# Aditya-Somasi/Vision-Inspection-System

Hardware: AMD Instinct MI355X
Metric: inspected images/sec (1024x1024, Qwen2-VL-7B) (higher is better)
Workload: dtype bf16; 1 GPU; configs[1]: Qwen2-VL-7B Inspector bf16, single 1024x1024 image per step per GPU, greedy decode 128 tok; batch=1, image_px=1024, weights=seeded random bf16 at exact 7B shapes, parallelism=dp1 (whole images)

## Files before the change

### include/vis_hip.h

```cpp
#ifndef VIS_HIP_H
#define VIS_HIP_H

#ifdef __cplusplus
extern "C" {
#endif

typedef void* vis_stream_t;

#define VIS_OK 0
#define VIS_ERR_ARG 1
#define VIS_ERR_LAUNCH 2
#define VIS_ERR_UNSUPPORTED 3

#define VIS_ACT_NONE 0
#define VIS_ACT_QUICKGELU 1
#define VIS_ACT_GELU_ERF 2
#define VIS_ACT_SWIGLU 3

int vis_abi_version(void);

int vis_gemm_bf16(const void* A, const void* W, const void* bias, const void* R, void* C,
                  int M, int N, int K, int lda, int ldw, int ldc, int ldr, int act, vis_stream_t stream);

int vis_rmsnorm_bf16(const void* x, const void* w, void* y, int rows, int N, int ldx, int ldy,
// ... 53 lines not shown

int vis_decode_attn_parts(const void* part, int ksplit, int slab_rows, const void* bias, const void* sx, const void* sw,
                          const void* cos_t, const void* sin_t, void* k_cache, void* v_cache, const void* step_ptr,
                          void* part_o, void* part_ml, void* out, int Hq, int Hkv, int HD, int cache_tokens, int nsplit,
                          float scale, int batch, long long cache_bs, long long tab_bs, int shared_len, vis_stream_t stream);

int vis_decode_attn_forked(const void* qkv, const void* cos_t, const void* sin_t, void* k_cache, void* v_cache,
                           const void* step_ptr, void* part_o, void* part_ml, void* out, int Hq, int Hkv, int HD,
                           int cache_tokens, int nsplit, float scale, int batch, long long qkv_bs, long long cache_bs,
                           long long tab_bs, const int* parent, const int* fork_len, vis_stream_t stream);
int vis_decode_attn_parts_forked(const void* part, int ksplit, int slab_rows, const void* bias, const void* sx, const void* sw,
                                 const void* cos_t, const void* sin_t, void* k_cache, void* v_cache, const void* step_ptr,
                                 void* part_o, void* part_ml, void* out, int Hq, int Hkv, int HD, int cache_tokens, int nsplit,
                                 float scale, int batch, long long cache_bs, long long tab_bs, const int* parent,
                                 const int* fork_len, vis_stream_t stream);

int vis_decode_chain_sync_ints(void);
long long vis_decode_chain_ws_bytes(int Hq, int Hkv, int nsplit);
int vis_decode_chain_ctx_limit(int Hq, int Hkv, int K);
int vis_decode_chain(const void* x, const void* x_idx, int x_rows, const void* Wqkv, const void* bqkv, const void* norm_w, const void* Wo, void* y,
                     const void* cos_t, const void* sin_t, void* k_cache, void* v_cache, const void* step_ptr,
                     void* ws, void* sync, int Hq, int Hkv, int HD, int K, int ldw_qkv, int ldw_o,
                     int cache_tokens, int nsplit, int ctx_bound, float scale, float eps, vis_stream_t stream);

int vis_gemv_bf16_argmax(const void* x, const void* W, const void* norm_w, void* logits, int N, int K, int ldw, float eps,
                         void* ws_val, void* ws_idx, void* tokens, int max_tokens, void* cur_token, void* step_ptr,
                         float inv_temp, unsigned seed, vis_stream_t stream);

int vis_argmax_f32(const void* logits, int V, void* ws_val, void* ws_idx, void* tokens, int max_tokens,
                   void* cur_token, void* step_ptr, float inv_temp, unsigned seed, int batch, int ld_logits,
                   vis_stream_t stream);

long long vis_logprobs_ws_bytes(int V, int batch);
int vis_logprobs_f32(const void* logits, int V, int ld_logits, const void* tokens, int max_tokens, const void* step_ptr,
                     int top_k, void* lp, void* top_ids, void* ws, long long ws_bytes, int batch, vis_stream_t stream);

int vis_json_mask(void* state, const void* tokens, int max_tokens, const void* step_ptr, const void* tok_off,
                  const void* tok_bytes, const void* tok_flags, const void* eos_ids, int n_eos, int V, void* allow,
                  int ld_allow, int batch, vis_stream_t stream);
int vis_schema_mask(void* state, const void* tokens, int max_tokens, const void* step_ptr, const void* tok_off,
                    const void* tok_bytes, const void* tok_flags, const void* eos_ids, int n_eos, int V, void* allow,
                    int ld_allow, const void* header, const void* trans, const void* byte_class, const void* state_flags,
                    int cap_states, int cap_classes, int batch, vis_stream_t stream);
int vis_argmax_masked_f32(const void* logits, int V, void* ws_val, void* ws_idx, void* tokens, int max_tokens,
                          void* cur_token, void* step_ptr, float inv_temp, unsigned seed, int batch, int ld_logits,
                          const void* allow, int ld_allow, vis_stream_t stream);
// ... 212 lines not shown
```

### vision-inspection-system_amd/decode_stage.py

```python
from __future__ import annotations

import logging
import os
import threading
from typing import Dict, List, NamedTuple, Optional, Sequence

import torch

from . import hip, spec
from .fork import check_fork_tables, fork_layout
from .pick import PickStage

_LOG = logging.getLogger("vision_inspection_system_amd.engine")

_CHAIN_LOCKS_GUARD = threading.Lock()
_CHAIN_ORDER_LOCKS: Dict[Optional[int], threading.Lock] = {}
_CHAIN_LAST: Dict[Optional[int], "torch.cuda.Event"] = {}


def _chain_order_lock(index: Optional[int]) -> threading.Lock:
    with _CHAIN_LOCKS_GUARD:
        return _CHAIN_ORDER_LOCKS.setdefault(index, threading.Lock())


class DecodeLayer(NamedTuple):
    w: object
    q8: Optional[dict]
    q4: Optional[dict]
    cross: bool
    idx: int
    bias: Optional[torch.Tensor]


_GEMV = {"bf16": "gemv", "fp8": "gemv_fp8", "mxfp4": "gemv_mxfp4"}


def _wt(L: DecodeLayer, name: str, fmt: str) -> tuple:
    return (getattr(L.w, name),) if fmt == "bf16" else (L.q8 if fmt == "fp8" else L.q4)[name]


class DecodeStage(PickStage):

    def _init_decode_stage(self, layers: Sequence[DecodeLayer], norm_w: torch.Tensor, lm_head: torch.Tensor,
                           q8_head: Optional[tuple] = None, q4_head: Optional[tuple] = None) -> None:
        self.dec_layers: List[DecodeLayer] = list(layers)
        self.dec_norm_w = norm_w
        self.dec_head = {"bf16": (lm_head,), "fp8": q8_head, "mxfp4": q4_head}
        self.dec_n_self = sum(1 for L in self.dec_layers if not L.cross)
        self._init_pick_stage()
        self.fork_on = False
        self.fork_parent_b: Optional[torch.Tensor] = None
        self.fork_len_b: Optional[torch.Tensor] = None
        self._spec: Optional[spec.SpecBuffers] = None
        self._spec_cfg: Optional[spec.SpecConfig] = None
        self._spec_pred = False
        self._spec_graphs: Dict[tuple, torch.cuda.CUDAGraph] = {}

    def _attn_share(self, B: int, shared: int) -> dict:
        if self.fork_on:
            return dict(fork=(self.fork_parent_b[:B], self.fork_len_b[:B]))
        return dict(shared_len=shared)

    def _fork_model_state(self, root: int, child: int) -> None:
        """Hook: copy what the model keeps per slot besides the self KV cache (rope rows, cross-attention keys) from ``root``
        into ``child``."""

    def _fork_choices(self, roots: Sequence[Optional[int]], n: Sequence[int], prefix_len: int, seeds, penalties,
                      shaping) -> List[Optional[List[int]]]:
        live = [j for j in range(len(roots)) if roots[j] is not None]
        lay = fork_layout([self.slot_prompt_len[roots[j]] for j in live], [n[j] for j in live], prefix_len, self.max_batch)
        out: List[Optional[List[int]]] = [None] * len(roots)
        for i, j in enumerate(live):
            if roots[j] != i:
                raise RuntimeError("prompt passes did not fill consecutive slots")
            out[j] = lay.slots[i]
        for child, root, lo, hi in lay.copies:
            j = live[root]
            self.kcache_b[child][:, :, lo:hi].copy_(self.kcache_b[root][:, :, lo:hi])
            self.vcache_b[child][:, :, lo:hi].copy_(self.vcache_b[root][:, :, lo:hi])
# ... 86 lines not shown
                    continue
                q = qkv[..., :Hq * D]
                proj(x, _wt(L, "qkv_w", fmt), q, norm_w=lw.ln1_w, eps=eps)
                self._decode_cross_attn(L, q, att, B)
                proj(att, _wt(L, "o_w", fmt), x2, residual=x)
            else:
                kc, vc = (self.kcache_b[:B, L.idx], self.vcache_b[:B, L.idx]) if B else (self.kcache[L.idx], self.vcache[L.idx])
                if chained:
                    try:
                        hip.decode_chain(self.w.embed if li == 0 else x, lw.qkv_w, L.bias, lw.ln1_w, lw.o_w, x2, cos, sin, kc, vc,
                                         step, self.chain_ws, self.chain_sync, Hq, Hkv, D, self.nsplit, scale, eps,
                                         x_index=cur if li == 0 else None, ctx_bound=self.chain_ctx_limit)
                    except hip.ChainRefused as e:
                        if li:
                            raise
                        _LOG.warning("%s - decoding on the four launches per layer head (VIS_MAX_CTX=%d)", e, self.max_ctx)
                        self.chain_sync, self._chain_state, chained = None, None, False
                        hip.gather_rows(self.w.embed, cur, self.d_x)
                if not chained:
                    proj(x, _wt(L, "qkv_w", fmt), qkv, bias=L.bias, norm_w=lw.ln1_w, eps=eps)
                    hip.decode_attn(qkv, cos, sin, kc, vc, step, self.part_o, self.part_ml, att, Hq, Hkv, D, self.nsplit, scale,
                                    **(self._attn_share(B, shared) if B else {}))
                    proj(att, _wt(L, "o_w", fmt), x2, residual=x)
            proj(x2, _wt(L, "gateup_w", fmt), act, norm_w=lw.ln2_w, act=hip.ACT_SWIGLU, eps=eps)
            proj(act, _wt(L, "down_w", fmt), x, residual=x2)
        if chained:
            self._gemv_pick(x, *self.dec_head["bf16"], logits, self.ws_val, self.ws_idx, tokens, cur, step,
                            norm_w=self.dec_norm_w, eps=eps, temperature=self.temperature, seed=self.seed)
        else:
            proj(x, self.dec_head[fmt], logits, norm_w=self.dec_norm_w, eps=eps)
            self._pick(logits, self.ws_val, self.ws_idx, tokens, cur, step, self.temperature, self.seed)
        self._logprobs_after_pick(B or 1)
        self._stop_after_pick(B or 1)
        self._stream_after_pick(B or 1)

    def _spec_begin(self, cfg: "spec.SpecConfig", max_new_tokens: int,
                    prediction: Optional[Sequence[int]] = None) -> "spec.SpecBuffers":
        cross = self.dec_n_self != len(self.dec_layers)
        if cross and not self.speculative_supported:
            raise ValueError("speculative decoding is not supported on a model with cross-attention layers unless its engine "
                             "was built for it (MllamaEngine(.., speculative=True))")
        spec.check_rows_fit(self.cfg, cfg.rows)
        if cross:
            spec.check_cross_rows_fit(self.cfg, cfg.rows)
        if self._spec is None:
            self._spec = spec.SpecBuffers(self.cfg, max(self.nsplit, self.xsplit) if cross else self.nsplit, self.max_ctx,
# ... 265 lines not shown
        g = torch.cuda.CUDAGraph()
        with torch.cuda.graph(g, capture_error_mode="thread_local"):
            step_fn()
        if len(cache) >= capacity:
            cache.pop(next(iter(cache)))
        cache[key] = g
        return g

    def _decode_steps(self, n_steps: int, use_graph: bool, chained: bool = False) -> None:
        if use_graph:
            g = self._ensure_graph(chained=chained)
            if chained and self.chain_sync is None:
                g = self._ensure_graph(chained=False)
            for _ in range(n_steps):
                g.replay()
        else:
            for _ in range(n_steps):
                self._decode_step(chained)

    def _decode_ordered(self, n_steps: int, use_graph: bool) -> None:
        base = self.prompt_len + self._decoded
        self._decoded += n_steps
        n_chain = max(0, min(n_steps, self.chain_ctx_limit - base)) if self.chain_sync is not None else 0
        if n_chain:
            self._chain_epoch_guard(n_chain)
            with _chain_order_lock(self.device.index):
                cur = torch.cuda.current_stream(self.device)
                prev = _CHAIN_LAST.get(self.device.index)
                if prev is not None:
                    cur.wait_event(prev)
                self._decode_steps(n_chain, use_graph, True)
                ev = torch.cuda.Event()
                ev.record(cur)
                _CHAIN_LAST[self.device.index] = ev
        if n_steps > n_chain:
            self._decode_steps(n_steps - n_chain, use_graph, False)

    def _chain_epoch_guard(self, n_steps: int) -> None:
        self._chain_launches += n_steps * self.dec_n_self
        if self._chain_launches >= (1 << 31):
            self.chain_sync.zero_()
            self.chain_ws.zero_()
            self._chain_launches = n_steps * self.dec_n_self

    def generated(self, n: int) -> List[int]:
        s = self.prompt_len - 1
        toks = self.tokens[s:s + n].cpu().tolist()
        self.check_chain()
        return toks

    def check_chain(self) -> None:
        if self.chain_sync is not None and int(self.chain_sync[hip.CHAIN_STATUS_WORD].item()) != 0:
            self.chain_sync.zero_()
            self.chain_ws.zero_()
            self._chain_launches = 0
            raise hip.ChainStalled("vis_decode_chain: a hand-off wait inside the launch timed out (decode results invalid)")
```

### vision-inspection-system_amd/engine.py

```python
from __future__ import annotations

import collections
import logging
import os
import threading
from typing import Dict, List, Optional, Sequence, Tuple

import numpy as np
import torch

from . import hip
from .decode_stage import DecodeLayer
from .generation import Generation
from .request import Switches
from .config import Qwen2VLConfig
from .weights import DeviceWeights, PATCH_K_PAD


def _round_up(x: int, m: int) -> int:
    return (x + m - 1) // m * m


def vision_pos_hw(grids: Sequence[Tuple[int, int, int]], merge: int) -> np.ndarray:
    out = []
# ... 788 lines not shown
    def shared_prefix_len(self, id_lists: Sequence[Sequence[int]]) -> int:
        if len(id_lists) < 2 or os.environ.get("VIS_SHARE_PREFIX", "1") == "0":
            return 0
        cfg = self.cfg
        first = np.asarray(list(id_lists[0]), dtype=np.int64)
        P = len(first) - 1
        for ids in id_lists[1:]:
            other = np.asarray(list(ids), dtype=np.int64)
            m = min(P, len(other) - 1)
            neq = np.nonzero(first[:m] != other[:m])[0]
            P = int(neq[0]) if neq.size else m
        special = np.nonzero((first[:P] == cfg.image_token_id) | (first[:P] == cfg.vision_start_id))[0]
        if special.size:
            P = int(special[0])
        P = (P // 64) * 64
        return P if P >= self.min_shared_prefix else 0

    def _decode_rope(self, B: int) -> tuple:
        return self.cos_b[:B], self.sin_b[:B], self.batch_shared_len

    def _ensure_graph(self, batch: int = 0, chained: bool = False) -> torch.cuda.CUDAGraph:
        fork = bool(batch) and self.fork_on
        key = (self.temperature, self.seed, batch, self.batch_shared_len if batch and not fork else 0,
               bool(chained) and not batch, fork) + self._pick_key() + self._stop_key() + self._shape_key() + self._stream_key() + self._ban_key()
        return self._captured_step(self._graphs, 8, key, batch, chained)

    def decode(self, n_steps: int, use_graph: bool = True) -> None:
        if self.prompt_len + n_steps + 1 > self.max_ctx:
            raise ValueError("decode would overflow the KV cache")
        if self.prompt_len + self._decoded + n_steps > self.decode_limit:
            raise ValueError("decode beyond the rope rows prepared by prefill (pass max_new_tokens)")
        self._decode_ordered(n_steps, use_graph)

    def disable_chain(self) -> None:
        if self.chain_sync is not None:
            self._chain_state = (self.chain_ws, self.chain_sync)
        self.chain_sync = None
        self._chain_clean_requests = 0
        self._graphs.clear()

    def _maybe_reenable_chain(self) -> None:
        if self.chain_sync is not None or self._chain_state is None:
            return
        self._chain_clean_requests += 1
        retry_after = int(os.environ.get("VIS_CHAIN_RETRY_AFTER", "64"))
        if retry_after > 0 and self._chain_clean_requests >= retry_after:
            self.chain_ws, self.chain_sync = self._chain_state
# ... 42 lines not shown
```

### vision-inspection-system_amd/generation.py

```python
from __future__ import annotations

import logging
from dataclasses import replace
from typing import List, Sequence

import torch

from . import hip, spec
from .ban import check_ban
from .decode_stage import DecodeStage
from .fork import check_n_list
from .json_mode import JsonModeError, check_schema
from .logprobs import check_k
from .penalties import check_penalties
from .request import Switches
from .sampling import check_seeds, check_top_p
from .shaping import check_shaping
from .stop import check_stop

_LOG = logging.getLogger("vision_inspection_system_amd.engine")


class Generation(DecodeStage):

# ... 23 lines not shown
        pred = spec.check_prediction_ids(sw.prediction, getattr(self, "max_ctx", None))
        sp = spec.with_prediction(sw.speculative, pred is not None)
        if sp is not None:
            what = "speculative" if pred is None else "prediction (speculative decoding)"
            if not self.speculative_supported:
                raise ValueError(("speculative decoding is" if pred is None else "prediction (speculative decoding) is") +
                                 " offered by the Qwen2-VL / Qwen2.5-VL engine only, unless an MllamaEngine is built for it: "
                                 "MllamaEngine(.., speculative=True), or VIS_AUDITOR_SPECULATIVE=k (1..3) where the client "
                                 "loads it")
            spec.check_exclusive(sp, temperature, seed, what=what, **sw.exclusive())
        penalties = check_penalties(sw.repetition_penalty, sw.frequency_penalty, sw.presence_penalty, 1)
        shaping = check_shaping(sw.top_k, sw.min_p, sw.logit_bias, 1)
        ban = check_ban(sw.no_repeat_ngram_size, sw.bad_words, sw.min_tokens, 1, max_new_tokens, json_mode=sw.json_mode,
                        json_schema=sw.json_schema)
        with self._pick_request(sw.logprobs, sw.json_mode, sw.json_schema, sw.top_p, False, penalties, stop=sw.stop,
                                shaping=shaping, on_stream=sw.on_stream, **({} if ban is None else {"ban": ban})):
            self.stop_eos = not ignore_eos
            self._stream_bind([[0]])
            max_new_tokens = self._clamp_request(input_ids, max_new_tokens)
            if sp is not None:
                return self._run_single_spec(sp, input_ids, frames, max_new_tokens, ignore_eos, use_graph, check_every, pred, temperature, seed)
            try:
                out = self._run_single(input_ids, frames, max_new_tokens, ignore_eos, use_graph, check_every, temperature, seed)
                self._maybe_reenable_chain()
                return out
            except hip.ChainStalled as e:
                _LOG.warning("%s - continuing on the unchained decode step", e)
                self.disable_chain()
                return self._run_single(input_ids, frames, max_new_tokens, ignore_eos, use_graph, check_every, temperature, seed)

    def _run_single(self, input_ids, frames, max_new_tokens, ignore_eos, use_graph, check_every, temperature, seed) -> List[int]:
        ev = [torch.cuda.Event(enable_timing=True) for _ in range(3)]
        ev[0].record()
        self._prompt_pass(input_ids, frames, max_new_tokens, temperature, seed)
        ev[1].record()
        max_new_tokens = min(max_new_tokens, self.max_ctx - len(input_ids) - 1)
        done, eos = 1, set(self.cfg.eos_ids)
        while done < max_new_tokens and not self._stream_cancelled():
            if self.stop_on:
                if self._stop_done([0]):
                    break
            elif not ignore_eos and any(t in eos for t in self.generated(done)):
                break
            n = min(check_every if not ignore_eos or self.stop_on else max_new_tokens, max_new_tokens - done)
            self.decode(n, use_graph=use_graph)
            done += n
        ev[2].record()
# ... 157 lines not shown
```

### vision-inspection-system_amd/hip.py

```python
from __future__ import annotations

import ctypes
import os
from typing import Optional, Sequence

import torch

_CSRC = os.path.join(os.path.dirname(os.path.abspath(__file__)), "csrc")
LIB_PATH = os.environ.get("VIS_HIP_LIB") or os.path.join(_CSRC, "libvis_hip.so")

ACT_NONE, ACT_QUICKGELU, ACT_GELU_ERF, ACT_SWIGLU = 0, 1, 2, 3
DECODE_KEYS_PER_SPLIT = 64

_SIGS = {
    "vis_abi_version": "",
    "vis_gemm_bf16": "ppppp" + "iiiiiiii" + "p",
    "vis_gemm_bf16_splitk": "pppppp" + "iiiiiiiii" + "p",
    "vis_gemm_bf16_splitk_part": "ppp" + "iiiiii" + "p",
    "vis_splitk_finalize_norm": "p" + "i" + "pppppp" + "iiiii" + "f" + "p",
    "vis_gemm_fp8": "pppppppp" + "iiiiiiiii" + "p",
    "vis_gemm_bf16_plan": "iiiiiiii" + "p" + "i",
    "vis_gemm_fp8_plan": "iiiiiiiii" + "p" + "i",
    "vis_quant_rows_fp8": "ppppp" + "iiii" + "f" + "p",
    "vis_rmsnorm_bf16": "ppp" + "iiii" + "f" + "p",
# ... 5 lines not shown
    "vis_attn_prefill_rows": "ppppp" + "iiiiiiiii" + "f" + "i" + "p",
    "vis_attn_prefill_rows_many": "ppppp" + "iiiiiiiii" + "f" + "i" + "i" + "lll" + "p" + "p",
    "vis_attn_prefill_pairs": "ppppp" + "iiiiiiii" + "f" + "i" + "p",
    "vis_attn_prefill_pairs_many": "ppppp" + "iiiiiiii" + "f" + "i" + "i" + "lll" + "p" + "p",
    "vis_attn_split_ws_bytes": "ii",
    "vis_attn_prefill_split": "ppppp" + "iiiiiiii" + "f" + "i" + "p" + "l" + "p",
    "vis_gemv_bf16": "pppppp" + "iiiii" + "f" + "p",
    "vis_gemv_fp8w": "ppppppp" + "iiiii" + "f" + "p",
    "vis_gemv_bf16_rows": "pppppp" + "iiiiiiiii" + "f" + "p",
    "vis_gemv_fp8w_rows": "ppppppp" + "iiiiiiiii" + "f" + "p",
    "vis_gemv_mxfp4w": "ppppppp" + "iiiiii" + "f" + "p",
    "vis_gemv_mxfp4w_rows": "ppppppp" + "iiiiiiiiii" + "f" + "p",
    "vis_gemm_decode_mxfp4_ksplit": "ii",
    "vis_gemm_decode_mxfp4": "ppppp" + "iiiiiiiii" + "p",
    "vis_decode_attn": "ppppppppp" + "iiiii" + "f" + "i" + "lll" + "p",
    "vis_decode_attn_shared": "ppppppppp" + "iiiii" + "f" + "i" + "lll" + "i" + "p",
    "vis_decode_attn_parts": "p" + "ii" + "p" * 11 + "iiiii" + "f" + "i" + "ll" + "i" + "p",
    "vis_decode_attn_forked": "ppppppppp" + "iiiii" + "f" + "i" + "lll" + "pp" + "p",
    "vis_decode_attn_parts_forked": "p" + "ii" + "p" * 11 + "iiiii" + "f" + "i" + "ll" + "pp" + "p",
    "vis_decode_chain_sync_ints": "",
    "vis_decode_chain_ws_bytes": "iii",
    "vis_decode_chain_ctx_limit": "iii",
    "vis_decode_chain": "ppi" + "p" * 12 + "i" * 9 + "ff" + "p",
    "vis_gemv_bf16_argmax": "pppp" + "iii" + "f" + "ppp" + "i" + "pp" + "fu" + "p",
    "vis_argmax_f32": "p" + "i" + "ppp" + "i" + "pp" + "fu" + "ii" + "p",
    "vis_logprobs_ws_bytes": "ii",
    "vis_logprobs_f32": "p" + "ii" + "p" + "i" + "p" + "i" + "ppp" + "l" + "i" + "p",
    "vis_json_mask": "pp" + "i" + "p" * 5 + "iip" + "ii" + "p",
    "vis_schema_mask": "pp" + "i" + "p" * 5 + "iip" + "i" + "pppp" + "iii" + "p",
    "vis_argmax_masked_f32": "p" + "i" + "ppp" + "i" + "pp" + "fu" + "ii" + "p" + "i" + "p",
    "vis_gemv_bf16_argmax_masked": "pppp" + "iii" + "f" + "ppp" + "i" + "pp" + "fu" + "p" + "p",
    "vis_sample_ws_bytes": "ii",
    "vis_sample_f32": "p" + "ii" + "p" + "i" + "ff" + "pp" + "i" + "pp" + "i" + "pp" + "p",
    "vis_penalty_state_bytes": "ii",
    "vis_penalty_prompt": "pi" + "pi" + "p",
    "vis_penalize_f32": "p" + "ii" + "ppp" + "i" + "pp" + "ii" + "p",
    "vis_shape_ws_bytes": "ii",
    "vis_shape_f32": "p" + "ii" + "p" + "i" + "ppppp" + "p" + "i" + "pp" + "i" + "p",
    "vis_ban_f32": "p" + "ii" + "p" + "i" + "pp" + "i" + "pppppp" + "i" + "p" + "i" + "p" + "ii" + "p",
    "vis_decode_attn_draft": "ppppppppp" + "iiiii" + "f" + "i" + "l" + "p",
    "vis_decode_cross_attn_draft": "pppppppp" + "iiiii" + "ff" + "il" + "p",
    "vis_decode_cross_attn_fp8_draft": "pppppppppp" + "iiiii" + "ff" + "il" + "p",
    "vis_spec_accept": "p" + "iii" + "pppppp" + "i" + "ppp" + "p",
    "vis_spec_accept_sampled": "p" + "iii" + "pppppp" + "i" + "ppp" + "p" + "p",
    "vis_spec_accept_masked": "p" + "iii" + "pppppp" + "i" + "ppp" + "p" + "pi" + "p",
    "vis_schema_mask_rows": "pp" + "i" + "ppp" + "i" + "pppp" + "ii" + "p" + "i" + "pppp" + "ii" + "p",
# ... 113 lines not shown
    global _CALL_TRACE
    tr, _CALL_TRACE = _CALL_TRACE, None
    return tr or {}


def exported_symbols() -> list:
    return list(_SIGS)


def load() -> ctypes.CDLL:
    global _lib
    if _lib is not None:
        return _lib
    if not os.path.exists(LIB_PATH):
        raise HipLibraryError(
            f"{LIB_PATH} not found: build it with `make -C {_CSRC}` (or __graft_entry__.build()); "
            "this package has no CPU fallback")
    lib = ctypes.CDLL(LIB_PATH)
    for name, sig in _SIGS.items():
        fn = getattr(lib, name)
        fn.restype = ctypes.c_int
        fn.argtypes = [_CT[c] for c in sig]
    lib.vis_decode_chain_ws_bytes.restype = ctypes.c_longlong
    lib.vis_decode_proj_ws_bytes.restype = ctypes.c_longlong
    lib.vis_logprobs_ws_bytes.restype = ctypes.c_longlong
    lib.vis_sample_ws_bytes.restype = ctypes.c_longlong
    lib.vis_penalty_state_bytes.restype = ctypes.c_longlong
    lib.vis_shape_ws_bytes.restype = ctypes.c_longlong
    _lib = _Lib(lib)
    return _lib


def _check(rc: int, name: str) -> None:
    if rc != 0:
        why = {1: "argument/shape/alignment precondition violated", 2: "HIP launch error",
               3: "shape not covered by this kernel form on this device"}.get(rc, "unknown")
        raise HipLibraryError(f"{name} failed with status {rc} ({why})")


def _ptr(t: Optional[torch.Tensor]) -> Optional[int]:
    if t is None:
        return None
    if not t.is_cuda:
        raise HipLibraryError("device tensor required (no CPU path exists)")
    return t.data_ptr()

# ... 810 lines not shown
    if qkv_w.shape != (nq, K) or qkv_w.stride(1) != 1 or o_w.shape != (K, n_q * head_dim) or o_w.stride(1) != 1 \
            or norm_w.numel() != K or y.numel() != K or (qkv_b is not None and qkv_b.numel() != nq):
        raise HipLibraryError("decode_chain: bad projection shapes")
    if k_cache.dim() != 3 or k_cache.shape[0] != n_kv or k_cache.shape[2] != head_dim or v_cache.shape != k_cache.shape \
            or not k_cache.is_contiguous() or not v_cache.is_contiguous():
        raise HipLibraryError("decode_chain: bad cache shape")
    T = k_cache.shape[1]
    if cos_t.shape != (T, head_dim) or sin_t.shape != cos_t.shape or cos_t.dtype != torch.float32 or not cos_t.is_contiguous() \
            or not sin_t.is_contiguous() or step.dtype != torch.int32 or step.numel() != 1:
        raise HipLibraryError("decode_chain: bad tables / step")
    lib = load()
    if ws.dtype != torch.int64 or ws.numel() * 8 < lib.vis_decode_chain_ws_bytes(n_q, n_kv, nsplit) \
            or sync.dtype != torch.int32 or sync.numel() < lib.vis_decode_chain_sync_ints():
        raise HipLibraryError("decode_chain: workspace too small")
    rc = lib.vis_decode_chain(_ptr(x), _ptr(x_index), x_rows, _ptr(qkv_w), _ptr(qkv_b), _ptr(norm_w), _ptr(o_w), _ptr(y), _ptr(cos_t), _ptr(sin_t),
                              _ptr(k_cache), _ptr(v_cache), _ptr(step), _ptr(ws), _ptr(sync), n_q, n_kv, head_dim, K,
                              qkv_w.stride(0), o_w.stride(0), T, nsplit, ctx_bound, scale, eps, _stream())
    if rc == 3:
        raise ChainRefused(f"vis_decode_chain: {n_q}/{n_kv} heads, hidden {K}, {nsplit} context splits are outside the chained "
                           "form on this device (shape, or grid larger than the device holds resident); nothing was launched")
    _check(rc, "vis_decode_chain")


def decode_chain_rows(ws: torch.Tensor, n_q: int, n_kv: int):
    nq = (n_q + 2 * n_kv) * 64
    g = ws[:nq + n_q * 64] & 0xFFFFFFFF
    rows = g.to(torch.int32).view(torch.bfloat16)
    return rows[:2 * nq], rows[2 * nq:]


def gemv_argmax(x: torch.Tensor, w: torch.Tensor, logits: torch.Tensor, ws_val: torch.Tensor, ws_idx: torch.Tensor,
                tokens: torch.Tensor, cur_token: torch.Tensor, step: torch.Tensor, norm_w: Optional[torch.Tensor] = None,
                eps: float = 1e-6, temperature: float = 0.0, seed: int = 0) -> None:
    _bf16(x, "gemv_argmax x"); _bf16(w, "gemv_argmax w")
    N, K = w.shape
    if x.numel() != K or w.stride(1) != 1 or logits.dtype != torch.float32 or logits.numel() != N:
        raise HipLibraryError("gemv_argmax: bad shapes")
    if ws_val.dtype != torch.float32 or ws_idx.dtype != torch.int32 or ws_val.numel() < 2048 or ws_idx.numel() < 2048 \
            or tokens.dtype != torch.int32 or cur_token.numel() != 1 or step.numel() != 1 or not tokens.is_contiguous():
        raise HipLibraryError("gemv_argmax: workspace too small / bad state shapes")
    rc = load().vis_gemv_bf16_argmax(_ptr(x), _ptr(w), _ptr(norm_w), _ptr(logits), N, K, w.stride(0), eps, _ptr(ws_val),
                                     _ptr(ws_idx), _ptr(tokens), tokens.numel(), _ptr(cur_token), _ptr(step),
                                     (1.0 / temperature) if temperature > 0 else 0.0, seed & 0xFFFFFFFF, _stream())
    _check(rc, "vis_gemv_bf16_argmax")


# ... 1005 lines not shown
```

Measured before the change: 2.641 images/s.

## Fuse decode MLP into one persistent kernel with LDS DMA weight ring

Adds a persistent decode MLP kernel that runs RMSNorm, gate/up GEMV with SwiGLU, a grid-wide hand-off of the activation through tagged global granules, and the down GEMV with residual inside a single launch. One loader wave streams weight rows into an LDS ring with buffer-load-to-LDS while three consumer waves compute. The decode step uses it for bf16 single-sequence decoding and falls back to the two GEMV launches otherwise. The aim is to remove per-layer launch overhead and the round trip between the two MLP GEMVs. In exchange it adds spin-wait synchronisation that depends on all blocks being resident, epoch bookkeeping, and timeout fallback paths.

```diff
diff --git a/include/vis_hip.h b/include/vis_hip.h
--- a/include/vis_hip.h
+++ b/include/vis_hip.h
@@ -99,6 +99,14 @@
                      const void* cos_t, const void* sin_t, void* k_cache, void* v_cache, const void* step_ptr,
                      void* ws, void* sync, int Hq, int Hkv, int HD, int K, int ldw_qkv, int ldw_o,
                      int cache_tokens, int nsplit, int ctx_bound, float scale, float eps, vis_stream_t stream);
+
+int vis_decode_mlp_sync_ints(void);
+long long vis_decode_mlp_ws_bytes(int I);
+int vis_decode_mlp_slot_chunks(void);
+int vis_decode_mlp_ring_slots(void);
+int vis_decode_mlp_supported(int H, int I);
+int vis_decode_mlp(const void* x2, const void* norm_w, const void* Wgu, const void* Wd, void* act, void* y, void* ws,
+                   void* sync, int H, int I, int ldw_gu, int ldw_d, float eps, vis_stream_t stream);
 
 int vis_gemv_bf16_argmax(const void* x, const void* W, const void* norm_w, void* logits, int N, int K, int ldw, float eps,
                          void* ws_val, void* ws_idx, void* tokens, int max_tokens, void* cur_token, void* step_ptr,
diff --git a/vision-inspection-system_amd/csrc/decode_mlp.hip b/vision-inspection-system_amd/csrc/decode_mlp.hip
--- /dev/null
+++ b/vision-inspection-system_amd/csrc/decode_mlp.hip
@@ -0,0 +1,315 @@
+#include "decode_common.hip.h"
+#include "attn_tile_dma.hip.h"
+#include "decode_mlp_plan.h"
+
+#define DM_EPOCH 0
+#define DM_STATUS 32
+#define DM_INTS 64
+
+struct MlpArgs {
+  const bf16_t* x2;
+  const bf16_t* norm_w;
+  const bf16_t* Wgu;
+  const bf16_t* Wd;
+  bf16_t* act;
+  bf16_t* y;
+  gran_t* act_g;
+  int* sync;
+  int H, I, ldw_gu, ldw_d;
+  float eps;
+  unsigned long long* probe;
+};
+
+#ifdef DMLP_PROBE
+#define DM_STAMP(i) do { if (lane == 0 && p.probe) p.probe[(size_t)blockIdx.x * 8 + (i)] = wall_clock64(); } while (0)
+#else
+#define DM_STAMP(i) do { } while (0)
+#endif
+
+__device__ __forceinline__ void dm_wait_vm(int n) {
+  switch (n >> 1) {
+#define DM_VM(k) case k: asm volatile("s_waitcnt vmcnt(%0)" ::"n"(2 * k) : "memory"); break;
+    DM_VM(0) DM_VM(1) DM_VM(2) DM_VM(3) DM_VM(4) DM_VM(5) DM_VM(6) DM_VM(7) DM_VM(8) DM_VM(9) DM_VM(10) DM_VM(11)
+    DM_VM(12) DM_VM(13) DM_VM(14) DM_VM(15)
+#undef DM_VM
+    default: asm volatile("s_waitcnt vmcnt(32)" ::: "memory"); break;
+  }
+}
+
+typedef __attribute__((address_space(3))) volatile unsigned dm_flag_t;
+typedef __attribute__((address_space(3))) char dm_lds_char;
+struct DmFlags {
+  dm_flag_t* full;
+  dm_flag_t* freed;
+  dm_flag_t* cbar;
+  dm_flag_t* dead;
+};
+#define DM_FLAG_WORDS (2 * DM_DEPTH + 2)
+
+__device__ __forceinline__ bool dm_wait_lds(dm_flag_t* w, unsigned want, int* status, const DmFlags& F) {
+  for (int it = 0; it < GV_CHAIN_SPIN_MAX; ++it) {
+    if (*w >= want) return true;
+    if (gr_poll_abort(status, it) || *F.dead) break;
+    __builtin_amdgcn_s_sleep(1);
+  }
+  *F.dead = 1u;
+  __hip_atomic_store(status, 1, __ATOMIC_RELAXED, __HIP_MEMORY_SCOPE_AGENT);
+  return false;
+}
+
+struct DmLoader {
+  int pos;
+  int pub;
+  int k_prev;
+};
+
+__device__ __forceinline__ void dm_publish(DmLoader& L, const DmFlags& F, int upto, int lane) {
+  if (lane == 0)
+    for (int q = L.pub; q <= upto; ++q) F.full[q % DM_DEPTH] = (unsigned)(q / DM_DEPTH) + 1u;
+  if (upto >= L.pub) L.pub = upto + 1;
+}
+
+__device__ __forceinline__ bool dm_load_phase(DmLoader& L, const DmFlags& F, const DmPhase& ph, bool swiglu, const bf16_t* W, int n_rows,
+                                              int ldw, dm_lds_char* ring, int lane, int* status) {
+  const uint32_t nrec = (uint32_t)n_rows * (uint32_t)ldw * 2u;
+  const __amdgpu_buffer_rsrc_t rs = __builtin_amdgcn_make_buffer_rsrc((void*)W, 0, (int)nrec, 0x00020000);
+  for (int R = 0; R * DM_NCONS < ph.n_units; ++R) {
+    const int left = ph.n_units - R * DM_NCONS, m = left < DM_NCONS ? left : DM_NCONS;
+    for (int sub = 0; sub < ph.spu; ++sub) {
+      const int pi = sub / ph.nseg, seg = sub - pi * ph.nseg;
+      const int js = min(DM_SLOT_J, ph.nj - seg * DM_SLOT_J);
+      for (int w = 0; w < m; ++w) {
+        const int slot = L.pos % DM_DEPTH, gen = L.pos / DM_DEPTH;
+        if (gen > 0 && F.freed[slot] < (unsigned)gen) {
+          dm_wait_vm(0);
+          dm_publish(L, F, L.pos - 1, lane);
+          L.k_prev = 0;
+          if (!dm_wait_lds(&F.freed[slot], (unsigned)gen, status, F)) return false;
+        }
+        int r0, r1;
+        dm_rows(swiglu, (ph.unit0 + R * DM_NCONS + w) * ph.ppu + pi, r0, r1);
+        dm_lds_char* dst = ring + slot * DM_SLOT_BYTES;
+        for (int i = 0; i < js; ++i) {
+          const int j = seg * DM_SLOT_J + i;
+          const uint32_t voff = (lane + 64 * j < ph.nch) ? (uint32_t)lane * 16u : nrec;
+          __builtin_amdgcn_raw_ptr_buffer_load_lds(rs, (att_lds_void*)(dst + i * 1024), 16, voff, r0 * ldw * 2 + j * 1024, 0, 2);
+          __builtin_amdgcn_raw_ptr_buffer_load_lds(rs, (att_lds_void*)(dst + DM_SLOT_BYTES / 2 + i * 1024), 16, voff,
+                                                   r1 * ldw * 2 + j * 1024, 0, 2);
+        }
+        dm_wait_vm(2 * js + L.k_prev);
+        dm_publish(L, F, L.pos - 2, lane);
+        L.k_prev = 2 * js;
+        ++L.pos;
+      }
+    }
+  }
+  return true;
+}
+
+template <bool SWIGLU>
+__device__ __forceinline__ bool dm_consume_phase(const MlpArgs& p, const DmFlags& F, const DmPhase& ph, int base, int cw, const bf16_t* xs,
+                                                 const dm_lds_char* ring, int lane, unsigned tag, int* status) {
+  for (int u = cw; u < ph.n_units; u += DM_NCONS) {
+    uint32_t first = 0;
+    for (int pi = 0; pi < ph.ppu; ++pi) {
+      float a0 = 0.f, a1 = 0.f;
+      for (int seg = 0; seg < ph.nseg; ++seg) {
+        const int pos = base + dm_pos(ph, u, pi * ph.nseg + seg);
+        const int slot = pos % DM_DEPTH, gen = pos / DM_DEPTH;
+        if (!dm_wait_lds(&F.full[slot], (unsigned)gen + 1u, status, F)) return false;
+        asm volatile("" ::: "memory");
+        const dm_lds_char* src = ring + slot * DM_SLOT_BYTES + lane * 16;
+        u32x4 w0[DM_SLOT_J], w1[DM_SLOT_J], xv[DM_SLOT_J];
+#pragma unroll
+        for (int i = 0; i < DM_SLOT_J; ++i) {
+          const int c = lane + 64 * (seg * DM_SLOT_J + i);
+          w0[i] = *(const __attribute__((address_space(3))) u32x4*)(src + i * 1024);
+          w1[i] = *(const __attribute__((address_space(3))) u32x4*)(src + DM_SLOT_BYTES / 2 + i * 1024);
+          xv[i] = *(const u32x4*)(xs + (size_t)min(c, ph.nch - 1) * 8);
+        }
+        asm volatile("s_waitcnt lgkmcnt(0)" ::: "memory");
+        if (lane == 0) F.freed[slot] = (unsigned)gen + 1u;
+#pragma unroll
+        for (int i = 0; i < DM_SLOT_J; ++i) {
+          const int c = lane + 64 * (seg * DM_SLOT_J + i);
+          if (c < ph.nch) {
+            a0 = dot8(w0[i], xv[i], a0);
+            a1 = dot8(w1[i], xv[i], a1);
+          }
+        }
+      }
+      a0 = wave_sum(a0);
+      a1 = wave_sum(a1);
+      const int pair = (ph.unit0 + u) * ph.ppu + pi;
+      if (lane == 0) {
+        if (SWIGLU) {
+          const bf16_t v = f2bf(silu_fast(a0) * a1);
+          p.act[pair] = v;
+          if (pi == 0) first = v;
+          else gr_st(p.act_g + (ph.unit0 + u), first | ((uint32_t)v << 16), tag);
+        } else {
+          const int o = 2 * pair;
+          float v0 = a0, v1 = a1;
+          v0 += bf2f(p.x2[o]);
+          v1 += bf2f(p.x2[o + 1]);
+          p.y[o] = f2bf(v0);
+          p.y[o + 1] = f2bf(v1);
+        }
+      }
+    }
+  }
+  return true;
+}
+
+__device__ __forceinline__ bool dm_sweep(const MlpArgs& p, const DmFlags& F, uint32_t* act_s, int cw, int lane, unsigned tag, int* status) {
+  constexpr int NST = 16;
+  const int ng = p.I >> 1;
+  const int per = ((ng + DM_NCONS - 1) / DM_NCONS + 63) & ~63;
+  const int g0 = cw * per, g1 = min(g0 + per, ng);
+  for (int base = g0; base < g1; base += 64 * NST) {
+    gran_t g[NST];
+    bool ok = false;
+    for (int it = 0; it < GV_CHAIN_SPIN_MAX && !ok; ++it) {
+#pragma unroll
+      for (int k = 0; k < NST; ++k) g[k] = gr_ld(p.act_g + min(base + lane + 64 * k, g1 - 1));
+      ok = true;
+#pragma unroll
+      for (int k = 0; k < NST; ++k)
+        if (base + lane + 64 * k < g1 && !gr_ok(g[k], tag)) ok = false;
+      ok = __all(ok);
+      if (!ok) {
+        if (gr_poll_abort(status, it) || *F.dead) break;
+        __builtin_amdgcn_s_sleep(2);
+      }
+    }
+    if (!ok) {
+      *F.dead = 1u;
+      __hip_atomic_store(status, 1, __ATOMIC_RELAXED, __HIP_MEMORY_SCOPE_AGENT);
+      return false;
+    }
+#pragma unroll
+    for (int k = 0; k < NST; ++k)
+      if (base + lane + 64 * k < g1) act_s[base + lane + 64 * k] = (uint32_t)g[k];
+  }
+  return true;
+}
+
+__global__ __launch_bounds__(256) void decode_mlp_kernel(MlpArgs p) {
+  extern __shared__ __attribute__((aligned(1024))) char smem[];
+  __shared__ unsigned flag_words[DM_FLAG_WORDS];
+  dm_flag_t* fw = (dm_flag_t*)flag_words;
+  const DmFlags F{fw, fw + DM_DEPTH, fw + 2 * DM_DEPTH, fw + 2 * DM_DEPTH + 1};
+  const int tid = threadIdx.x, lane = tid & 63, wave = tid >> 6;
+  const int b = blockIdx.x, G = gridDim.x;
+  const unsigned e = (unsigned)__hip_atomic_load(p.sync + DM_EPOCH, __ATOMIC_RELAXED, __HIP_MEMORY_SCOPE_AGENT);
+  const unsigned tag = (e + 1u != 0u) ? e + 1u : 1u;
+  int* status = p.sync + DM_STATUS;
+  if (__hip_atomic_load(status, __ATOMIC_RELAXED, __HIP_MEMORY_SCOPE_AGENT) != 0) {
+    if (b == 0 && tid == 0) __hip_atomic_store(p.sync + DM_EPOCH, (int)tag, __ATOMIC_RELAXED, __HIP_MEMORY_SCOPE_AGENT);
+    return;
+  }
+  bf16_t* xs = (bf16_t*)smem;
+  const int xs_bytes = (p.H * 2 + 1023) / 1024 * 1024, as_bytes = (p.I * 2 + 1023) / 1024 * 1024;
+  uint32_t* act_s = (uint32_t*)(smem + xs_bytes);
+  dm_lds_char* ring = (dm_lds_char*)(smem + xs_bytes + as_bytes);
+  const DmPhase pa = dm_phase(p.I >> 1, 2, p.H, b, G);
+  const DmPhase pb = dm_phase(p.H >> 1, 1, p.I, b, G);
+  if (tid < DM_FLAG_WORDS) fw[tid] = 0u;
+  DM_STAMP(0);
+  gv_stage_x_rmsnorm(p.x2, p.norm_w, xs, p.H >> 3, p.H, p.eps, tid, lane, wave);
+  __syncthreads();
+
+  if (wave == 0) {
+    DmLoader L{0, 0, 0};
+    bool ok = dm_load_phase(L, F, pa, true, p.Wgu, 2 * p.I, p.ldw_gu, ring, lane, status);
+    DM_STAMP(1);
+    ok = ok && dm_load_phase(L, F, pb, false, p.Wd, p.H, p.ldw_d, ring, lane, status);
+    dm_wait_vm(0);
+    if (ok) dm_publish(L, F, L.pos - 1, lane);
+    DM_STAMP(2);
+    return;
+  }
+
+  const int cw = wave - 1;
+  bool ok = dm_consume_phase<true>(p, F, pa, 0, cw, xs, ring, lane, tag, status);
+  if (cw == 0) DM_STAMP(3);
+  ok = ok && dm_sweep(p, F, act_s, cw, lane, tag, status);
+  asm volatile("s_waitcnt lgkmcnt(0)" ::: "memory");
+  if (lane == 0)
+    __hip_atomic_fetch_add((__attribute__((address_space(3))) unsigned*)F.cbar, 1u, __ATOMIC_RELEASE, __HIP_MEMORY_SCOPE_WORKGROUP);
+  if (ok) ok = dm_wait_lds(F.cbar, (unsigned)DM_NCONS, status, F);
+  __builtin_amdgcn_fence(__ATOMIC_ACQUIRE, "workgroup");
+  if (cw == 0) DM_STAMP(4);
+  ok = ok && !*F.dead;
+  if (ok) ok = dm_consume_phase<false>(p, F, pb, dm_total_slots(pa), cw, (const bf16_t*)act_s, ring, lane, tag, status);
+  if (cw == 0) DM_STAMP(5);
+  if (b == 0 && cw == 0 && lane == 0) __hip_atomic_store(p.sync + DM_EPOCH, (int)tag, __ATOMIC_RELAXED, __HIP_MEMORY_SCOPE_AGENT);
+}
+
+#define DM_MAX_DEVICES 16
+static int mlp_resident_blocks(size_t lds) {
+  struct Entry { size_t lds; int blocks; bool attr_set; };
+  static Entry cache[DM_MAX_DEVICES] = {};
+  int dev = 0;
+  if (hipGetDevice(&dev) != hipSuccess || dev < 0 || dev >= DM_MAX_DEVICES) return 0;
+  Entry& en = cache[dev];
+  if (!en.attr_set) {
+    if (hipFuncSetAttribute((const void*)decode_mlp_kernel, hipFuncAttributeMaxDynamicSharedMemorySize, (int)(156 * 1024)) != hipSuccess)
+      return 0;
+    en.attr_set = true;
+  }
+  if (en.lds == lds && en.blocks > 0) return en.blocks;
+  hipFuncAttributes fa;
+  if (hipFuncGetAttributes(&fa, (const void*)decode_mlp_kernel) != hipSuccess) return 0;
+  int cus = 0;
+  if (hipDeviceGetAttribute(&cus, hipDeviceAttributeMultiprocessorCount, dev) != hipSuccess) return 0;
+  const int vg = ((fa.numRegs > 0 ? fa.numRegs : 512) + 7) / 8 * 8;
+  int per_simd = 512 / vg;
+  if (per_simd > 8) per_simd = 8;
+  const int by_lds = (int)((160 * 1024) / (lds + fa.sharedSizeBytes + 256));
+  const int per_cu = per_simd < by_lds ? per_simd : by_lds;
+  en.lds = lds;
+  en.blocks = per_cu * cus;
+  return en.blocks;
+}
+
+static unsigned long long* g_mlp_probe = nullptr;
+#ifdef DMLP_PROBE
+extern "C" void vis_decode_mlp_set_probe(void* p) { g_mlp_probe = (unsigned long long*)p; }
+#endif
+
+extern "C" int vis_decode_mlp_sync_ints(void) { return DM_INTS; }
+
+extern "C" long long vis_decode_mlp_ws_bytes(int I) { return I > 0 ? (long long)sizeof(gran_t) * ((I + 1) / 2) : 0; }
+
+extern "C" int vis_decode_mlp_slot_chunks(void) { return DM_SLOT_CHUNKS; }
+extern "C" int vis_decode_mlp_ring_slots(void) { return DM_DEPTH; }
+
+extern "C" int vis_decode_mlp_supported(int H, int I) {
+  if (!dm_shape_ok(H, I, H, I)) return 0;
+  return mlp_resident_blocks((size_t)dm_lds_bytes(H, I)) >= 1 ? 1 : 0;
+}
+
+extern "C" int vis_decode_mlp(const void* x2, const void* norm_w, const void* Wgu, const void* Wd, void* act, void* y, void* ws,
+                              void* sync, int H, int I, int ldw_gu, int ldw_d, float eps, hipStream_t stream) {
+  if (!x2 || !norm_w || !Wgu || !Wd || !act || !y || !ws || !sync || H <= 0 || I <= 0) return VIS_ERR_ARG;
+  if (((uintptr_t)x2 | (uintptr_t)norm_w | (uintptr_t)Wgu | (uintptr_t)Wd) & 15) return VIS_ERR_ARG;
+  if ((((uintptr_t)act | (uintptr_t)y | (uintptr_t)sync) & 3) || ((uintptr_t)ws & 7)) return VIS_ERR_ARG;
+  if (!dm_shape_ok(H, I, ldw_gu, ldw_d)) return VIS_ERR_UNSUPPORTED;
+  const size_t lds = (size_t)dm_lds_bytes(H, I);
+  if (lds > 156 * 1024) return VIS_ERR_UNSUPPORTED;
+  const int resident = mlp_resident_blocks(lds);
+  int cus = 0, dev = 0;
+  if (hipGetDevice(&dev) != hipSuccess || hipDeviceGetAttribute(&cus, hipDeviceAttributeMultiprocessorCount, dev) != hipSuccess)
+    return VIS_ERR_LAUNCH;
+  const int grid = resident < cus ? resident : cus;
+  if (grid < 1) return VIS_ERR_UNSUPPORTED;
+  MlpArgs p;
+  p.x2 = (const bf16_t*)x2; p.norm_w = (const bf16_t*)norm_w; p.Wgu = (const bf16_t*)Wgu; p.Wd = (const bf16_t*)Wd;
+  p.act = (bf16_t*)act; p.y = (bf16_t*)y; p.act_g = (gran_t*)ws; p.sync = (int*)sync;
+  p.H = H; p.I = I; p.ldw_gu = ldw_gu; p.ldw_d = ldw_d; p.eps = eps;
+  p.probe = g_mlp_probe;
+  vis_clear_error();
+  hipLaunchKernelGGL(decode_mlp_kernel, dim3(grid), dim3(256), lds, stream, p);
+  return vis_check_launch();
+}
diff --git a/vision-inspection-system_amd/csrc/decode_mlp_plan.h b/vision-inspection-system_amd/csrc/decode_mlp_plan.h
--- /dev/null
+++ b/vision-inspection-system_amd/csrc/decode_mlp_plan.h
@@ -0,0 +1,66 @@
+#pragma once
+
+#if defined(__HIPCC__)
+#define DM_HD __host__ __device__ __forceinline__
+#else
+#define DM_HD static inline
+#endif
+
+#define DM_NCONS 3
+#define DM_SLOT_J 8
+#define DM_SLOT_CHUNKS (DM_SLOT_J * 64)
+#define DM_SLOT_BYTES (2 * DM_SLOT_CHUNKS * 16)
+#define DM_DEPTH 6
+#define DM_MAX_H 4096
+#define DM_MAX_I 20480
+#define DM_FLAG_BYTES 256
+
+struct DmPhase {
+  int unit0;
+  int n_units;
+  int ppu;
+  int nch;
+  int nj;
+  int nseg;
+  int spu;
+};
+
+DM_HD int dm_share_begin(int n_units, int b, int G) { return (int)((long long)n_units * b / G); }
+
+DM_HD DmPhase dm_phase(int n_units_total, int ppu, int K, int b, int G) {
+  DmPhase ph;
+  ph.unit0 = dm_share_begin(n_units_total, b, G);
+  ph.n_units = dm_share_begin(n_units_total, b + 1, G) - ph.unit0;
+  ph.ppu = ppu;
+  ph.nch = K >> 3;
+  ph.nj = (ph.nch + 63) >> 6;
+  ph.nseg = (ph.nj + DM_SLOT_J - 1) / DM_SLOT_J;
+  ph.spu = ppu * ph.nseg;
+  return ph;
+}
+
+DM_HD int dm_total_slots(const DmPhase& ph) { return ph.n_units * ph.spu; }
+
+DM_HD int dm_pos(const DmPhase& ph, int u, int sub) {
+  const int R = u / DM_NCONS, w = u - R * DM_NCONS;
+  const int left = ph.n_units - R * DM_NCONS;
+  const int m = left < DM_NCONS ? left : DM_NCONS;
+  return R * DM_NCONS * ph.spu + sub * m + w;
+}
+
+DM_HD void dm_rows(bool swiglu, int pair, int& r0, int& r1) {
+  if (swiglu) { r0 = ((pair >> 4) << 5) + (pair & 15); r1 = r0 + 16; }
+  else { r0 = 2 * pair; r1 = r0 + 1; }
+}
+
+DM_HD long long dm_lds_bytes(int H, int I) {
+  const long long xs = ((long long)H * 2 + 1023) / 1024 * 1024, as = ((long long)I * 2 + 1023) / 1024 * 1024;
+  return xs + as + (long long)DM_DEPTH * DM_SLOT_BYTES;
+}
+
+DM_HD bool dm_shape_ok(int H, int I, long long ldw_gu, long long ldw_d) {
+  if (H < 64 || I < 32 || H % 8 != 0 || I % 16 != 0 || H > DM_MAX_H || I > DM_MAX_I) return false;
+  if (ldw_gu < H || ldw_d < I || ldw_gu % 8 != 0 || ldw_d % 8 != 0) return false;
+  if (2LL * I * ldw_gu * 2 >= (1LL << 30) || (long long)H * ldw_d * 2 >= (1LL << 30)) return false;
+  return true;
+}
diff --git a/vision-inspection-system_amd/decode_stage.py b/vision-inspection-system_amd/decode_stage.py
--- a/vision-inspection-system_amd/decode_stage.py
+++ b/vision-inspection-system_amd/decode_stage.py
@@ -16,6 +16,9 @@
 _CHAIN_LOCKS_GUARD = threading.Lock()
 _CHAIN_ORDER_LOCKS: Dict[Optional[int], threading.Lock] = {}
 _CHAIN_LAST: Dict[Optional[int], "torch.cuda.Event"] = {}
+
+
+MLP_LAUNCH_DEFAULT = False
 
 
 def _chain_order_lock(index: Optional[int]) -> threading.Lock:
@@ -47,6 +50,7 @@
         self.dec_norm_w = norm_w
         self.dec_head = {"bf16": (lm_head,), "fp8": q8_head, "mxfp4": q4_head}
         self.dec_n_self = sum(1 for L in self.dec_layers if not L.cross)
+        self._init_mlp_launch(getattr(self, "decode_weights", "") if self.dec_n_self == len(self.dec_layers) else "")
         self._init_pick_stage()
         self.fork_on = False
         self.fork_parent_b: Optional[torch.Tensor] = None
@@ -55,6 +59,42 @@
         self._spec_cfg: Optional[spec.SpecConfig] = None
         self._spec_pred = False
         self._spec_graphs: Dict[tuple, torch.cuda.CUDAGraph] = {}
+
+    def _init_mlp_launch(self, decode_weights: str) -> None:
+        self.mlp_sync: Optional[torch.Tensor] = None
+        self.mlp_ws: Optional[torch.Tensor] = None
+        self._mlp_state: Optional[tuple] = None
+        self._mlp_launches = 0
+        self._mlp_clean_requests = 0
+        env = os.environ.get("VIS_DECODE_MLP", "")
+        if decode_weights != "bf16" or env == "0" or (env == "" and not MLP_LAUNCH_DEFAULT):
+            return
+        H = self.cfg.hidden
+        on = env == "1" or (env == "" and MLP_LAUNCH_DEFAULT and
+                            H // 2 >= 3 * torch.cuda.get_device_properties(self.device).multi_processor_count)
+        if decode_weights == "bf16" and on and os.environ.get("VIS_DECODE_CHAIN", "1") != "0" \
+                and hip.decode_mlp_supported(H, self.cfg.intermediate):
+            self.mlp_ws, self.mlp_sync = hip.decode_mlp_state(self.device, self.cfg.intermediate)
+
+    def _mlp_disable(self) -> None:
+        if self.mlp_sync is not None:
+            self._mlp_state = (self.mlp_ws, self.mlp_sync)
+        self.mlp_sync = None
+
+    def _after_clean_request(self) -> None:
+        self._maybe_reenable_chain()
+        if self.mlp_sync is not None or self._mlp_state is None:
+            return
+        self._mlp_clean_requests += 1
+        retry_after = int(os.environ.get("VIS_CHAIN_RETRY_AFTER", "64"))
+        if retry_after > 0 and self._mlp_clean_requests >= retry_after:
+            self.mlp_ws, self.mlp_sync = self._mlp_state
+            self._mlp_state = None
+            self.mlp_sync.zero_()
+            self.mlp_ws.zero_()
+            self._mlp_launches = 0
+            _LOG.warning("vis_decode_mlp: %d requests served on the two GEMVs since the stall - persistent MLP launch back on",
+                         self._mlp_clean_requests)
 
     def _attn_share(self, B: int, shared: int) -> dict:
         if self.fork_on:
@@ -187,6 +227,15 @@
                     hip.decode_attn(qkv, cos, sin, kc, vc, step, self.part_o, self.part_ml, att, Hq, Hkv, D, self.nsplit, scale,
                                     **(self._attn_share(B, shared) if B else {}))
                     proj(att, _wt(L, "o_w", fmt), x2, residual=x)
+            if not B and fmt == "bf16" and self.mlp_sync is not None:
+                try:
+                    hip.decode_mlp(x2, lw.ln2_w, lw.gateup_w, lw.down_w, act, x, self.mlp_ws, self.mlp_sync, eps)
+                    continue
+                except hip.MlpRefused as e:
+                    if li:
+                        raise
+                    _LOG.warning("%s - decoding on the two GEMV launches per MLP", e)
+                    self.mlp_sync = self._mlp_state = None
             proj(x2, _wt(L, "gateup_w", fmt), act, norm_w=lw.ln2_w, act=hip.ACT_SWIGLU, eps=eps)
             proj(act, _wt(L, "down_w", fmt), x, residual=x2)
         if chained:
@@ -498,26 +547,36 @@
         base = self.prompt_len + self._decoded
         self._decoded += n_steps
         n_chain = max(0, min(n_steps, self.chain_ctx_limit - base)) if self.chain_sync is not None else 0
-        if n_chain:
-            self._chain_epoch_guard(n_chain)
+        waiting = n_steps if self.mlp_sync is not None else n_chain
+        if waiting:
+            self._chain_epoch_guard(n_chain, n_steps if self.mlp_sync is not None else 0)
             with _chain_order_lock(self.device.index):
                 cur = torch.cuda.current_stream(self.device)
                 prev = _CHAIN_LAST.get(self.device.index)
                 if prev is not None:
                     cur.wait_event(prev)
-                self._decode_steps(n_chain, use_graph, True)
+                if n_chain:
+                    self._decode_steps(n_chain, use_graph, True)
+                if waiting > n_chain:
+                    self._decode_steps(waiting - n_chain, use_graph, False)
                 ev = torch.cuda.Event()
                 ev.record(cur)
                 _CHAIN_LAST[self.device.index] = ev
-        if n_steps > n_chain:
-            self._decode_steps(n_steps - n_chain, use_graph, False)
-
-    def _chain_epoch_guard(self, n_steps: int) -> None:
+        if n_steps > waiting:
+            self._decode_steps(n_steps - waiting, use_graph, False)
+
+    def _chain_epoch_guard(self, n_steps: int, n_mlp_steps: int = 0) -> None:
         self._chain_launches += n_steps * self.dec_n_self
         if self._chain_launches >= (1 << 31):
             self.chain_sync.zero_()
             self.chain_ws.zero_()
             self._chain_launches = n_steps * self.dec_n_self
+        if n_mlp_steps:
+            self._mlp_launches += n_mlp_steps * len(self.dec_layers)
+            if self._mlp_launches >= (1 << 31):
+                self.mlp_sync.zero_()
+                self.mlp_ws.zero_()
+                self._mlp_launches = n_mlp_steps * len(self.dec_layers)
 
     def generated(self, n: int) -> List[int]:
         s = self.prompt_len - 1
@@ -531,3 +590,10 @@
             self.chain_ws.zero_()
             self._chain_launches = 0
             raise hip.ChainStalled("vis_decode_chain: a hand-off wait inside the launch timed out (decode results invalid)")
+        if self.mlp_sync is not None and int(self.mlp_sync[hip.CHAIN_STATUS_WORD].item()) != 0:
+            self.mlp_sync.zero_()
+            self.mlp_ws.zero_()
+            self._mlp_launches = 0
+            self._mlp_disable()
+            self._mlp_clean_requests = 0
+            raise hip.ChainStalled("vis_decode_mlp: a wait inside the persistent MLP launch timed out (decode results invalid)")
diff --git a/vision-inspection-system_amd/engine.py b/vision-inspection-system_amd/engine.py
--- a/vision-inspection-system_amd/engine.py
+++ b/vision-inspection-system_amd/engine.py
@@ -834,7 +834,7 @@
     def _ensure_graph(self, batch: int = 0, chained: bool = False) -> torch.cuda.CUDAGraph:
         fork = bool(batch) and self.fork_on
         key = (self.temperature, self.seed, batch, self.batch_shared_len if batch and not fork else 0,
-               bool(chained) and not batch, fork) + self._pick_key() + self._stop_key() + self._shape_key() + self._stream_key() + self._ban_key()
+               bool(chained) and not batch, fork, self.mlp_sync is not None and not batch) + self._pick_key() + self._stop_key() + self._shape_key() + self._stream_key() + self._ban_key()
         return self._captured_step(self._graphs, 8, key, batch, chained)
 
     def decode(self, n_steps: int, use_graph: bool = True) -> None:
diff --git a/vision-inspection-system_amd/generation.py b/vision-inspection-system_amd/generation.py
--- a/vision-inspection-system_amd/generation.py
+++ b/vision-inspection-system_amd/generation.py
@@ -69,7 +69,7 @@
                 return self._run_single_spec(sp, input_ids, frames, max_new_tokens, ignore_eos, use_graph, check_every, pred, temperature, seed)
             try:
                 out = self._run_single(input_ids, frames, max_new_tokens, ignore_eos, use_graph, check_every, temperature, seed)
-                self._maybe_reenable_chain()
+                self._after_clean_request()
                 return out
             except hip.ChainStalled as e:
                 _LOG.warning("%s - continuing on the unchained decode step", e)
diff --git a/vision-inspection-system_amd/hip.py b/vision-inspection-system_amd/hip.py
--- a/vision-inspection-system_amd/hip.py
+++ b/vision-inspection-system_amd/hip.py
@@ -51,6 +51,12 @@
     "vis_decode_chain_ws_bytes": "iii",
     "vis_decode_chain_ctx_limit": "iii",
     "vis_decode_chain": "ppi" + "p" * 12 + "i" * 9 + "ff" + "p",
+    "vis_decode_mlp_sync_ints": "",
+    "vis_decode_mlp_ws_bytes": "i",
+    "vis_decode_mlp_slot_chunks": "",
+    "vis_decode_mlp_ring_slots": "",
+    "vis_decode_mlp_supported": "ii",
+    "vis_decode_mlp": "p" * 8 + "iiii" + "f" + "p",
     "vis_gemv_bf16_argmax": "pppp" + "iii" + "f" + "ppp" + "i" + "pp" + "fu" + "p",
     "vis_argmax_f32": "p" + "i" + "ppp" + "i" + "pp" + "fu" + "ii" + "p",
     "vis_logprobs_ws_bytes": "ii",
@@ -210,6 +216,7 @@
         fn.restype = ctypes.c_int
         fn.argtypes = [_CT[c] for c in sig]
     lib.vis_decode_chain_ws_bytes.restype = ctypes.c_longlong
+    lib.vis_decode_mlp_ws_bytes.restype = ctypes.c_longlong
     lib.vis_decode_proj_ws_bytes.restype = ctypes.c_longlong
     lib.vis_logprobs_ws_bytes.restype = ctypes.c_longlong
     lib.vis_sample_ws_bytes.restype = ctypes.c_longlong
@@ -1066,6 +1073,42 @@
     _check(rc, "vis_decode_chain")
 
 
+class MlpRefused(HipLibraryError):
+    """vis_decode_mlp returned VIS_ERR_UNSUPPORTED: the MLP shape is outside the persistent form or the device cannot hold its
+    grid resident.  Nothing was launched; the caller issues the two GEMVs (same results bit for bit)."""
+
+
+def decode_mlp_state(device, intermediate: int):
+    lib = load()
+    nbytes = int(lib.vis_decode_mlp_ws_bytes(intermediate))
+    return (torch.zeros((nbytes + 7) // 8, dtype=torch.int64, device=device),
+            torch.zeros(lib.vis_decode_mlp_sync_ints(), dtype=torch.int32, device=device))
+
+
+def decode_mlp_supported(hidden: int, intermediate: int) -> bool:
+    return bool(load().vis_decode_mlp_supported(hidden, intermediate))
+
+
+def decode_mlp(x2: torch.Tensor, norm_w: torch.Tensor, gateup_w: torch.Tensor, down_w: torch.Tensor, act: torch.Tensor,
+               y: torch.Tensor, ws: torch.Tensor, sync: torch.Tensor, eps: float = 1e-6) -> torch.Tensor:
+    for n, t in (("x2", x2), ("norm_w", norm_w), ("gateup_w", gateup_w), ("down_w", down_w), ("act", act), ("y", y)):
+        _bf16(t, "decode_mlp " + n)
+    H, I = down_w.shape
+    if gateup_w.shape != (2 * I, H) or gateup_w.stride(1) != 1 or down_w.stride(1) != 1 or x2.numel() != H \
+            or norm_w.numel() != H or act.numel() != I or y.numel() != H or y.data_ptr() == x2.data_ptr():
+        raise HipLibraryError("decode_mlp: bad shapes")
+    lib = load()
+    if ws.dtype != torch.int64 or ws.numel() * 8 < lib.vis_decode_mlp_ws_bytes(I) or sync.dtype != torch.int32 \
+            or sync.numel() < lib.vis_decode_mlp_sync_ints():
+        raise HipLibraryError("decode_mlp: workspace too small")
+    rc = lib.vis_decode_mlp(_ptr(x2), _ptr(norm_w), _ptr(gateup_w), _ptr(down_w), _ptr(act), _ptr(y), _ptr(ws), _ptr(sync),
+                            H, I, gateup_w.stride(0), down_w.stride(0), eps, _stream())
+    if rc == 3:
+        raise MlpRefused(f"vis_decode_mlp: hidden {H}, intermediate {I} are outside the persistent MLP launch on this device")
+    _check(rc, "vis_decode_mlp")
+    return y
+
+
 def decode_chain_rows(ws: torch.Tensor, n_q: int, n_kv: int):
     nq = (n_q + 2 * n_kv) * 64
     g = ws[:nq + n_q * 64] & 0xFFFFFFFF
```

Result: no change. 2.640 images/s (-0.0%).
